# dymensionxyz/cometbft

Measured on AMD Instinct MI355X. Metric: Ed25519 verifs/sec at 1/2/4/8 GPUs + p50 VerifyCommit latency, 150 vals, higher is better.
Workload: dtype u32

## Files before the change

### cometbft_amd/csrc/hs_helper.h

```cpp
#pragma once
#include "devtables.h"
#include "quad.h"

namespace cmtv {

constexpr int kHsCombPre = 6, kHsCombPreFused = 3, kHsCombPreSr = 0;
constexpr uint32_t kHsSlotU2 = 3 * 5 * 64;
constexpr uint32_t kHsTabU2 = 2 * 9 * 5 * 64;

constexpr uint32_t kHsPsWords = 30;
constexpr int kHsFoldCombPre = 15;

__device__ __forceinline__ int hs_comb_pre(uint32_t hs_tune, int dflt) {
  const int c = (hs_tune & 0xFFu) ? (int)(hs_tune & 0xFFu) - 1 : dflt;
  return c > 16 ? 16 : c;
}

__device__ __forceinline__ int hs_workgroup_windows(uint32_t flags, uint32_t t) {
  const bool wide = __ballot(t < 48 && (flags & 2u) != 0) != 0;
  int W = HS_WINDOWS;
#pragma unroll 1
  for (int x = HS_WINDOWS; x < HS_MAX_WINDOWS; x++) W += __ballot(t < 48 && (int)((flags >> 8) & 0xFFu) > x) ? 1 : 0;
  return wide ? HS_WIDE_WINDOWS : W;
}
// ... 3 lines not shown
#pragma unroll
    for (int k = 0; k < 5; k++) dst[(t >> 4) * 320 + k * 64 + 4 * (t & 15) + c] = make_uint2(v.v[2 * k], v.v[2 * k + 1]);
  }
}

__device__ __forceinline__ void hs_slot_store(uint2* dst, uint32_t t, const fe* out) {
#pragma unroll
  for (int c = 0; c < 4; c++) hs_slot_store_coord(dst, t, c, out[c]);
}

struct HsWalk {
  uint32_t tA[8], tR[8];
  const uint2* tw;
  bool r_flip;
  __device__ __forceinline__ HsWalk(const SigPrep& p, int W, const uint2* tabs, uint32_t t) {
    const uint32_t slot = t < 48 ? t : 47;
    r_flip = (p.flags & 1u) != 0;
    hs_digits16(tA, p.k1, W);
    hs_digits16(tR, p.k2, W);
    sc_shift_out(tA, 4);
    sc_shift_out(tR, 4);
    tw = tabs + (slot >> 4) * kHsTabU2 + 4 * (slot & 15);
  }
  __device__ __forceinline__ void next(int& dA, int& dR) {
    dA = (int)sc_shift_out(tA, 4) - 8;
    dR = (int)sc_shift_out(tR, 4) - 8;
  }
  __device__ __forceinline__ void operator()(int P, int e, int c, fe& r) const {
    const uint2* src = tw + (P * 9 + e) * 5 * 64 + c;
#pragma unroll
    for (int k = 0; k < 5; k++) {
      const uint2 x = src[k * 64];
      r.v[2 * k] = x.x;
      r.v[2 * k + 1] = x.y;
    }
  }
};

template <class Clock>
__device__ __forceinline__ void hs_helper_sums(const SigPrep& p, int W, const uint2* tabs, uint2* ring, uint32_t t,
                                               const Clock& clock, uint64_t& hwait) {
  HsWalk rd(p, W, tabs, t);
#pragma unroll 1
  for (int win = W - 2; win >= 0; win--) {
    int dA, dR;
    rd.next(dA, dR);
    fe out[4];
    h_window_addend(out, rd, dA, dR, rd.r_flip);
    hs_slot_store(ring + (win & 1) * kHsSlotU2, t, out);
    const uint64_t c0 = clock();
    __syncthreads();
    hwait += clock() - c0;
  }
}

constexpr uint32_t kHsFgU2 = 2 * 5 * 48;
constexpr uint32_t kHsFgNone = 0xFFFFFFFFu;

__device__ __forceinline__ void hs_helper_sums_fg(const SigPrep& p, int W, const uint2* tabs, uint2* ring, uint2* fg,
                                                  uint32_t* fg_ready, uint32_t t) {
  HsWalk rd(p, W, tabs, t);
#pragma unroll 1
  for (int win = W - 2; win >= 0; win--) {
    int dA, dR;
    rd.next(dA, dR);
    fe z2, f, g;
    h_window_addend_fg(z2, f, g, rd, dA, dR, rd.r_flip);
    if (t < 48) {
#pragma unroll
      for (int k = 0; k < 5; k++) {
        fg[k * 48 + t] = make_uint2(f.v[2 * k], f.v[2 * k + 1]);
        fg[(5 + k) * 48 + t] = make_uint2(g.v[2 * k], g.v[2 * k + 1]);
      }
    }
    hs_slot_store_coord(ring + (win & 1) * kHsSlotU2, t, 2, z2);
    __builtin_amdgcn_fence(__ATOMIC_RELEASE, "workgroup");
    if (t == 0) __hip_atomic_store(fg_ready, (uint32_t)win, __ATOMIC_RELAXED, __HIP_MEMORY_SCOPE_WORKGROUP);
    __syncthreads();
  }
}

template <class Clock>
__device__ __forceinline__ bool hs_helper_sums_eh(const SigPrep& p, int W, const uint2* tabs, uint2* ring,
                                                  const uint2* fg, uint32_t* fg_ready, uint32_t fg_wait, uint32_t t,
                                                  const Clock& clock, uint64_t& hwait, uint64_t& fwait) {
  HsWalk rd(p, W, tabs, t);
  const uint32_t slot = t < 48 ? t : 47;
  bool late = false;
#pragma unroll 1
  for (int win = W - 2; win >= 0; win--) {
    int dA, dR;
    rd.next(dA, dR);
    uint2* dst = ring + (win & 1) * kHsSlotU2;
    fe out[4], e, h;
    h_window_addend_eh(out[3], e, h, rd, dA, dR, rd.r_flip);
    const uint64_t f0 = clock();
    bool ready = false;
    for (uint32_t spins = 0; spins < fg_wait; spins++) {
      ready = __hip_atomic_load(fg_ready, __ATOMIC_RELAXED, __HIP_MEMORY_SCOPE_WORKGROUP) == (uint32_t)win;
      if (ready) break;
      __builtin_amdgcn_s_sleep(1);
    }
    fwait += clock() - f0;
    if (__builtin_expect(__ballot(ready) != __ballot(1), 0)) {
      late = true;
      h_window_addend(out, rd, dA, dR, rd.r_flip);
// ... 48 lines not shown
```

### cometbft_amd/csrc/kernels.h

```cpp
#pragma once
#include <hip/hip_runtime.h>
#include <stdint.h>

namespace cmtv {

constexpr uint32_t kBtabWords = (3 * 128 + 3 * 32768 + 16 * 32768) * 36;
constexpr uint32_t kAtabWordsPerLane = 320;
constexpr uint32_t kCombWords = 32 * 128 * 32;
constexpr uint32_t kCombScratchWordsPerKey = 128 * 320;

constexpr uint32_t kFormLane = 0, kFormQuad = 1, kFormOct2 = 2, kFormRow = 3, kFormRow4 = 4;
constexpr uint32_t kFormMask = 0xFF, kLaunchForceWide = 0x100, kLaunchHsFold = 0x200;
constexpr uint32_t kHsTuneSumSplit = 1u << 11, kHsTuneFgLate = 1u << 12;
constexpr uint32_t kKeyedRow = 0, kKeyedQuad = 1, kKeyedLane = 2;

constexpr uint32_t kRowSlots = 256, kRowSlotWords = 1024, kRowMaxCap = 4 * (kRowSlotWords - 16);
struct RowSlot {
  uint32_t* words = nullptr;
  uint64_t* tagged = nullptr;
  uint32_t seq = 0;
};

struct SbFuse {
  const void* tmpls = nullptr;
  const uint8_t* blob = nullptr;
  const uint32_t* tidx = nullptr;
  const uint8_t* flag = nullptr;
  const int64_t* sec = nullptr;
  const int32_t* nanos = nullptr;
};
constexpr uint32_t kSbFuseMaxMsg = 192;

constexpr uint32_t kDiagLateK = 0, kDiagLatePs = 1, kDiagLateSum = 2, kDiagWords = 4;
constexpr uint32_t kKeyedWaitDefault = 1u << 22, kPsWaitDefault = 1u << 22;

hipError_t launch_btab_init(uint32_t* d_rows, hipStream_t s);
hipError_t launch_verify(uint32_t mode, uint32_t n, const void* pk, const void* sig, const void* msg,
                         const void* off, const uint32_t* btab, uint32_t* atab, void* valid, void* bitmap,
                         uint32_t kflags, hipStream_t s, const SbFuse* sb = nullptr, const RowSlot* row_slot = nullptr,
                         uint32_t ps_wait = kPsWaitDefault, uint32_t* diag = nullptr);
hipError_t launch_comb_build(uint32_t n_keys, const void* keys_pk, uint8_t* keys_ok, uint32_t* tabs,
                             uint32_t* scratch, bool negate, hipStream_t s);
hipError_t launch_verify_keyed(uint32_t mode, uint32_t n, uint32_t n_keys, const void* key_idx, const void* sig,
                               const void* msg, const void* off, const uint32_t* keys_pk, const uint8_t* keys_ok,
                               const uint32_t* ktabs, void* valid, void* bitmap, uint32_t form, uint32_t k_wait,
                               uint32_t* diag, uint32_t batch_kb, uint32_t* scr, const uint32_t* wtabs,
                               const uint32_t* btab, hipStream_t s, const RowSlot* row_slot = nullptr,
                               const SbFuse* sb = nullptr);
hipError_t launch_verify_keyed_lane(uint32_t mode, uint32_t n, uint32_t n_keys, const uint32_t* ki,
                                    const uint32_t* sgp, const uint8_t* mp, const uint32_t* op,
                                    const uint32_t* keys_pk, const uint8_t* keys_ok, const uint32_t* ktabs,
                                    uint8_t* vp, uint64_t* bp, uint32_t batch_kb, uint32_t* scr,
                                    const uint32_t* wtabs, const uint32_t* btab, hipStream_t s);
constexpr size_t kWideTableWords = (size_t)16 * 32768 * 32;
constexpr size_t kWideScratchWordsPerKey = (size_t)16 * (32768 / 64) * 64 * 10;
constexpr size_t kWideBaseWordsPerKey = 16 * 40;
hipError_t launch_wide_build(uint32_t n_keys, const void* keys_pk, uint32_t* tabs, uint32_t* bases,
                             uint32_t* scratch, hipStream_t s);
constexpr uint32_t kKeyedBatchScratchWordsPerSig = 40;
hipError_t launch_verify_sr25519(uint32_t n, const void* pk, const void* sig, const void* msg, const void* off,
                                 const uint32_t* btab, uint32_t* atab, const uint32_t* prog, int nops, void* valid,
                                 void* bitmap, uint32_t kflags, hipStream_t s);
constexpr uint32_t kSecpGtabWords = 33 * 128 * 32;
constexpr uint32_t kSecpQtabWordsPerLane = 240;
hipError_t launch_secp_gtab_build(uint32_t* d_rows, hipStream_t s);
hipError_t launch_verify_secp256k1(uint32_t n, const void* pk, const void* sig, const void* msg, const void* off,
// ... 53 lines not shown
```

### cometbft_amd/csrc/kernels.hip

```cpp
#include <hip/hip_runtime.h>

#include "devtables.h"
#include "hs_helper.h"
#include "kernel_parts.h"
#include "kernels.h"
#include "phase_probe.h"
#include "quad.h"
#include "signbytes.h"
#include "verify_core.h"

CMTV_PHASE_BUFFER()

#ifndef CMTV_QUAD_WAVES_PER_EU
#define CMTV_QUAD_WAVES_PER_EU 1
#endif

#ifndef CMTV_VERIFY_WAVES_PER_EU
#define CMTV_VERIFY_WAVES_PER_EU 2
#endif

namespace cmtv {

template <uint32_t MODE>
__global__ __launch_bounds__(64, CMTV_VERIFY_WAVES_PER_EU) void k_verify(uint32_t n, const uint32_t* __restrict__ pk,
// ... 42 lines not shown
                    [] { CMTV_STAMP(7); });
    const int W = hs_workgroup_windows(p.flags, t);
    p.flags |= (uint32_t)W << 16;
    if (t < 48) sig_prep_store(prep[t], p);
    BComb16 bc;
    bc.init(p.u);
    const DevBTab bt{btab};
#pragma unroll 1
    for (int k = 0; k < comb_pre; k++) bc.step(bt);
    CMTV_STAMP(1);
    __syncthreads();
    CMTV_STAMP(2);
    uint64_t hwait = 0;
    hs_helper_windows(p, W, bc, &tab_lds[0][0], xbuf, t, [] { return (uint64_t)CMTV_CLOCK(); }, hwait);
    CMTV_STAMP_VAL(6, hwait);
    CMTV_STAMP(3);
    __syncthreads();
    return;
  }
  const uint32_t ls = wave * 16 + (t >> 2);
  const uint32_t s = base + ls;
  const bool active = s < n;
  const uint32_t i = active ? s : n - 1;
  DevQuad q;
  DevATabQ ta{tab_lds[wave], t}, tr{tab_lds[wave] + 9 * 5 * 64, t};
  uint64_t qwait = 0;
  (void)qwait;
  DevBTabQ bt{btab};
  bool v = q_verify_hs<MODE>(
      q, pk + 8 * (size_t)i, sig + 16 * (size_t)i, bt, ta, tr, 16 - comb_pre,
      [&](SigPrep& p) {
        CMTV_STAMP(1);
        __syncthreads();
        CMTV_STAMP(2);
        sig_prep_load(p, prep[ls]);
      },
      [&](int win, fe& c) {
        const uint64_t c0 = CMTV_CLOCK();
        __syncthreads();
        qwait += CMTV_CLOCK() - c0;
        hs_slot_load(xbuf + (win & 1) * kHsSlotU2, wave, t, c);
      },
      [&](fe& c) {
        CMTV_STAMP(3);
        __syncthreads();
        CMTV_STAMP(4);
        hs_slot_load(xbuf + kHsSlotU2, wave, t, c);
      });
  CMTV_STAMP(5);
  CMTV_STAMP_VAL(6, qwait);
  quad_verdict_store(v, active, s, n, wave, t, out_valid, out_bitmap, tags);
}

template <uint32_t MODE>
__global__ __launch_bounds__(320, 1) void k_verify_quad_hs_fold(
    uint32_t n, const uint32_t* __restrict__ pk, const uint32_t* __restrict__ sig, const uint8_t* __restrict__ msg,
    const uint32_t* __restrict__ off, const uint32_t* __restrict__ btab, uint8_t* __restrict__ out_valid,
    uint64_t* __restrict__ out_bitmap, uint32_t force_wide, SbFuse sb, uint32_t hs_tune, uint32_t ps_wait,
    uint32_t* __restrict__ diag, RowSlot tags) {
  CMTV_URGENT();
  const uint32_t hw = threadIdx.x >> 6, t = threadIdx.x & 63;
  const uint32_t base = blockIdx.x * 48;
  const uint32_t tune = hs_tune >> 8;
  const int comb_pre = hs_comb_pre(hs_tune, kHsFoldCombPre);
  const uint32_t helper_wave = (tune & 1u) ? 3u : 0u;
  const bool sum_split = (hs_tune & kHsTuneSumSplit) != 0 && helper_wave == 0;
  const bool fg_late = (hs_tune & kHsTuneFgLate) != 0;
  __shared__ uint32_t prep[48][SIG_PREP_WORDS + 1];
  __shared__ uint2 tab_lds[3][kHsTabU2];
  __shared__ uint2 xbuf[2 * kHsSlotU2];
  __shared__ uint32_t ps_ready;
  __shared__ uint2 fgx[kHsFgU2];
  __shared__ uint32_t fg_ready;
  static_assert(sizeof(xbuf) >= 48 * (kSbFuseMaxMsg + 4 * kHsPsWords), "P_s goes behind the sign-bytes buffer");
  static_assert(sizeof(prep) + sizeof(tab_lds) + sizeof(xbuf) + sizeof(fgx) + 2 * sizeof(uint32_t) <= 160 * 1024,
                "a workgroup's LDS");
  uint32_t* pspt = reinterpret_cast<uint32_t*>(xbuf) + 48 * (kSbFuseMaxMsg / 4);
  CMTV_STAMP5(0);
  CMTV_HWID5();
  if (threadIdx.x == 0) {
    ps_ready = 0u;
    fg_ready = kHsFgNone;
  }
  __syncthreads();
  if (hw == 4) {
    if (tune & 2u) __builtin_amdgcn_s_setprio(0);
    if (tune & 4u) __builtin_amdgcn_s_setprio(3);
    if (ps_wait != 0) {
      const uint32_t slot = t < 48 ? t : 47;
      const uint32_t s = base + slot;
      const uint32_t i = s < n ? s : n - 1;
      uint32_t sw[8];
      load_words(sw, sig + 16 * (size_t)i + 8, 2);
      const DevBTab bt{btab};
      BComb16Ahead bc;
      bc.init(sw, bt);
#pragma unroll 1
      for (int k = 0; k < comb_pre; k++) bc.step(bt);
      if (t < 48) {
#pragma unroll
        for (int j = 0; j < 10; j++) {
          pspt[t * kHsPsWords + j] = bc.P.X.v[j];
          pspt[t * kHsPsWords + 10 + j] = bc.P.Y.v[j];
          pspt[t * kHsPsWords + 20 + j] = bc.P.Z.v[j];
        }
      }
      __builtin_amdgcn_fence(__ATOMIC_RELEASE, "workgroup");
      if (t == 0) __hip_atomic_store(&ps_ready, 1u, __ATOMIC_RELAXED, __HIP_MEMORY_SCOPE_WORKGROUP);
    }
    CMTV_STAMP5(3);
    CMTV_STAMP5(1);
    __syncthreads();
    CMTV_STAMP5(2);
    const int W = (int)__builtin_amdgcn_readfirstlane((prep[0][24] >> 16) & 0xFFu);
    if (sum_split && !fg_late) {
      SigPrep p;
      sig_prep_load_pair(p, prep[t < 48 ? t : 47]);
      hs_helper_sums_fg(p, W, &tab_lds[0][0], xbuf, fgx, &fg_ready, t);
      return;
    }
#pragma unroll 1
    for (int win = W - 2; win >= 0; win--) __syncthreads();
    return;
  }
  if (hw == helper_wave) {
    const uint32_t slot = t < 48 ? t : 47;
    const uint32_t s = base + slot;
    const uint32_t i = s < n ? s : n - 1;
    const uint8_t* mp;
    uint32_t ml;
    helper_message(sb, i, msg, off, reinterpret_cast<uint32_t*>(xbuf) + slot * (kSbFuseMaxMsg / 4), mp, ml);
    SigPrep p;
    q_prepare<MODE>(p, pk + 8 * (size_t)i, sig + 16 * (size_t)i, mp, ml, force_wide != 0);
    const int W = hs_workgroup_windows(p.flags, t);
    p.flags |= (uint32_t)W << 16;
    if (t < 48) sig_prep_store_pair(prep[t], p);
    CMTV_STAMP5(1);
    __syncthreads();
    CMTV_STAMP5(2);
    uint64_t hwait = 0, fwait = 0;
    (void)fwait;
    auto clock = [] { return (uint64_t)CMTV_CLOCK(); };
    if (sum_split) {
      const bool late = hs_helper_sums_eh(p, W, &tab_lds[0][0], xbuf, fgx, &fg_ready, fg_late ? 0u : kPsWaitDefault, t,
                                          clock, hwait, fwait);
      if (late && t == 0 && diag) atomicAdd(diag + kDiagLateSum, 1u);
    } else {
      hs_helper_sums(p, W, &tab_lds[0][0], xbuf, t, clock, hwait);
    }
    CMTV_STAMP5_VAL(4, fwait);
    CMTV_STAMP5_VAL(7, hwait);
    CMTV_STAMP5(3);
    return;
  }
  const uint32_t wave = hw - (hw > helper_wave ? 1u : 0u);
  const uint32_t ls = wave * 16 + (t >> 2);
  const uint32_t s = base + ls;
  const bool active = s < n;
  const uint32_t i = active ? s : n - 1;
  DevQuad q;
  DevATabQ ta{tab_lds[wave], t}, tr{tab_lds[wave] + 9 * 5 * 64, t};
  uint64_t qwait = 0;
  (void)qwait;
  bool v = q_verify_hs_fold<MODE>(
      q, pk + 8 * (size_t)i, sig + 16 * (size_t)i, DevBTabQ{btab}, 16 - comb_pre, ta, tr,
      [&](fe& ps) {
        const uint64_t c0 = CMTV_CLOCK();
        (void)c0;
        bool ready = false;
        for (uint32_t spins = 0; spins < ps_wait; spins++) {
          ready = __hip_atomic_load(&ps_ready, __ATOMIC_RELAXED, __HIP_MEMORY_SCOPE_WORKGROUP) != 0u;
          if (ready) break;
          __builtin_amdgcn_s_sleep(2);
        }
        CMTV_STAMP5_VAL(3, CMTV_CLOCK() - c0);
        if (__builtin_expect(__ballot(ready) != __ballot(1), 0)) {
          if (t == 0 && diag) atomicAdd(diag + kDiagLatePs, 1u);
          return false;
        }
        __builtin_amdgcn_fence(__ATOMIC_ACQUIRE, "workgroup");
        const int lane = (int)(t & 3);
        const uint32_t* pp = pspt + ls * kHsPsWords;
        fe a, b;
#pragma unroll
        for (int j = 0; j < 10; j++) {
          a.v[j] = pp[10 * q_p2_factor_a(lane) + j];
          b.v[j] = pp[10 * q_p2_factor_b(lane) + j];
        }
        fe_mul(ps, a, b);
        CMTV_STAMP5(4);
        return true;
      },
      [&](SigPrep& p) {
        CMTV_STAMP5(1);
        __syncthreads();
        CMTV_STAMP5(2);
        sig_prep_load_pair(p, prep[ls]);
      },
      [&](int win, fe& c) {
        const uint64_t c0 = CMTV_CLOCK();
        __syncthreads();
        qwait += CMTV_CLOCK() - c0;
        hs_slot_load(xbuf + (win & 1) * kHsSlotU2, wave, t, c);
      });
  CMTV_STAMP5(5);
  CMTV_STAMP5_VAL(7, qwait);
  quad_verdict_store(v, active, s, n, wave, t, out_valid, out_bitmap, tags);
}

template <uint32_t MODE>
__global__ __launch_bounds__(128, CMTV_QUAD_WAVES_PER_EU) void k_verify_oct_split(
    uint32_t n, const uint32_t* __restrict__ pk, const uint32_t* __restrict__ sig, const uint8_t* __restrict__ msg,
    const uint32_t* __restrict__ off, const uint32_t* __restrict__ btab, uint8_t* __restrict__ out_valid,
    uint64_t* __restrict__ out_bitmap, uint32_t force_wide, SbFuse sb) {
  CMTV_URGENT();
  const uint32_t t = threadIdx.x & 63;
  const uint32_t gid = blockIdx.x * 64 + t;
  const uint32_t s = gid >> 3;
  const bool active = s < n;
  const uint32_t i = active ? s : n - 1;
  __shared__ uint32_t prep[8][SIG_PREP_WORDS + 1];
  __shared__ uint32_t bpt[8][40];
  __shared__ uint2 tab_lds[9 * 5 * 64];
  __shared__ uint32_t sbm[8][kSbFuseMaxMsg / 4];
  if (threadIdx.x >= 64) {
    const uint8_t* mp;
    uint32_t ml;
    helper_message(sb, i, msg, off, sbm[t >> 3], mp, ml);
    SigPrep p;
    q_prepare<MODE>(p, pk + 8 * (size_t)i, sig + 16 * (size_t)i, mp, ml, force_wide != 0);
    if ((t & 7) == 0) sig_prep_store(prep[t >> 3], p);
    __syncthreads();
    ge_p3 B;
    q_bcomb16(B, p.u, DevBTab{btab});
    if ((t & 7) == 0) bpoint_store(bpt[t >> 3], B);
    __syncthreads();
    return;
  }
  DevOct q;
  DevBTabQ bt{btab};
  DevATabQ ta{tab_lds, t};
  const uint32_t* bq = &bpt[t >> 3][10 * (t & 3)];
  bool v = o_verify_split<MODE, true>(
      q, pk + 8 * (size_t)i, sig + 16 * (size_t)i, bt, ta,
      [&](SigPrep& p) {
        __syncthreads();
        sig_prep_load(p, prep[t >> 3]);
      },
      [&](fe& c) {
        __syncthreads();
#pragma unroll
        for (int j = 0; j < 10; j++) c.v[j] = bq[j];
      });
  v = v && active;
  if (active && (t & 7) == 0 && out_valid) out_valid[s] = v ? 1 : 0;
  uint64_t x = __ballot(v && (t & 7) == 0) & 0x0101010101010101ull;
  x = (x | (x >> 7)) & 0x0003000300030003ull;
  x = (x | (x >> 14)) & 0x0000000F0000000Full;
  x = (x | (x >> 28)) & 0xFFull;
  if (t == 0 && out_bitmap) reinterpret_cast<uint8_t*>(out_bitmap)[gid >> 6] = (uint8_t)x;
}

// ... 180 lines not shown
  const uint32_t limb = reinterpret_cast<const uint16_t*>(((t >> 4) & 1) ? sgp : pkp)[t & 15];
  DevRowTab tab{tab_lo, t};
  bool a_ok, r_ok, r_canon;
  const uint32_t v = r_sum_ar(x, limb, pkw, sigw, tab, get_prep, kRowLoWindows, p, a_ok, r_ok, r_canon);
  CMTV_STAMP(3);
  __syncthreads();
  CMTV_STAMP(4);
  const uint32_t cb = bpt_limb(bpt, t);
  bool v_ok = r_join4<MODE>(x, v, xh[0][t], xh[1][t], cb, (p.flags & 4u) != 0 && a_ok && r_ok, r_canon);
  CMTV_STAMP(5);
  CMTV_STAMP_RT(6);
  const bool active = s < n;
  v_ok = v_ok && active;
  if (t == 0 && active && out_valid) out_valid[s] = v_ok ? 1 : 0;
  if (out_bitmap && active) row_bitmap_add(slot, s, n, v_ok, out_bitmap, t);
}

hipError_t launch_verify(uint32_t mode, uint32_t n, const void* pk, const void* sig, const void* msg,
                         const void* off, const uint32_t* btab, uint32_t* atab, void* valid, void* bitmap,
                         uint32_t kflags, hipStream_t s, const SbFuse* sb, const RowSlot* row_slot, uint32_t ps_wait,
                         uint32_t* diag) {
  const SbFuse fz = sb ? *sb : SbFuse{};
  const uint32_t form = kflags & kFormMask;
  const uint32_t fw = (kflags & kLaunchForceWide) ? 1u : 0u;
  if (n == 0) return hipSuccess;
  auto pkp = static_cast<const uint32_t*>(pk);
  auto sgp = static_cast<const uint32_t*>(sig);
  auto mp = static_cast<const uint8_t*>(msg);
  auto op = static_cast<const uint32_t*>(off);
  auto vp = static_cast<uint8_t*>(valid);
  auto bp = static_cast<uint64_t*>(bitmap);
  const RowSlot rs = row_slot ? *row_slot : RowSlot{};
  if ((form == kFormRow4 || form == kFormRow) && (n > kRowMaxCap || (bp && !rs.words))) return hipErrorInvalidValue;
  if (form != kFormLane && form != kFormQuad && form != kFormOct2 && form != kFormRow && form != kFormRow4)
    return hipErrorInvalidValue;
  if (fz.tmpls && form == kFormLane) return hipErrorInvalidValue;
  with_mode(mode, [&](auto m) {
    constexpr uint32_t M = decltype(m)::value;
    switch (form) {
      case kFormRow4:
        hipLaunchKernelGGL(k_verify_row4_split<M>, dim3(n), dim3(256), 0, s, n, pkp, sgp, mp, op, btab, vp, bp, fw, fz,
                           rs);
        break;
      case kFormRow:
        hipLaunchKernelGGL(k_verify_row_split<M>, dim3((n + 2) / 3), dim3(256), 0, s, n, pkp, sgp, mp, op, btab, vp, bp,
                           fw, fz, rs);
        break;
      case kFormOct2:
        hipLaunchKernelGGL(k_verify_oct_split<M>, dim3(((n + 63) / 64) * 8), dim3(128), 0, s, n, pkp, sgp, mp, op, btab,
                           vp, bp, fw, fz);
        break;
      case kFormQuad: {
        const uint32_t slices = 4 * ((n + 63) / 64);
        if (kflags & kLaunchHsFold)
          hipLaunchKernelGGL(k_verify_quad_hs_fold<M>, dim3((slices + 2) / 3), dim3(320), 0, s, n, pkp, sgp, mp, op,
                             btab, vp, bp, fw, fz, kflags >> 16, ps_wait, diag, rs);
        else
          hipLaunchKernelGGL(k_verify_quad_hs<M>, dim3((slices + 2) / 3), dim3(256), 0, s, n, pkp, sgp, mp, op, btab,
                             vp, bp, fw, fz, kflags >> 16, rs);
        break;
      }
      default:
        hipLaunchKernelGGL(k_verify<M>, dim3((n + 63) / 64), dim3(64), 0, s, n, pkp, sgp, mp, op, btab, atab, vp, bp);
    }
  });
  return hipGetLastError();
}

}
```

### cometbft_amd/csrc/launch.cpp

```cpp
#include "runtime_state.h"

namespace cmtv {

struct LaunchScope {
  cmtv_ctx* ctx;
  CmtvDev& D;
  hipStream_t s;
  Timing::Pair tp{};
  bool timed = false;
  hipError_t begin() {
    D.timing.harvest(ctx->stats, D.device_ms, D.timed_calls, false);
    timed = ctx->timing_every && D.timing_seq++ % ctx->timing_every == 0;
    return timed ? D.timing.begin(tp, s) : hipSuccess;
  }
  hipError_t launched(hipError_t e) {
    if (e != hipSuccess) {
      D.timing.abandon(tp);
      return e;
    }
    ctx->stats.kernel_launches++;
    D.launches++;
    return hipSuccess;
  }
  int finish(size_t n, Scratch* lane_scratch) {
// ... 11 lines not shown
static void take_tags(CmtvDev& D, RowSlot& slot, uint32_t width) {
  slot.tagged = D.tag_arm;
  slot.seq = D.tag_seq;
  D.tag_used = true;
  D.tag_width = width;
}

bool fault_hit(cmtv_ctx* ctx) {
  ctx->launch_seq++;
  if (ctx->fault_at && ctx->launch_seq == ctx->fault_at) {
    ctx->stats.faults_injected++;
    ctx->fault_pending = true;
    return true;
  }
  return false;
}

static hipError_t row_slot_acquire(cmtv_ctx* ctx, CmtvDev& D, hipStream_t s, bool bitmap, RowSlot& slot,
                                   uint32_t& k) {
  hipError_t e0 = settle_polled(D);
  if (e0 != hipSuccess) return e0;
  k = D.row_seq++ % kRowSlots;
  slot = RowSlot{};
  slot.words = D.d_rowslots + (size_t)k * kRowSlotWords;
  if (bitmap && D.tag_arm) take_tags(D, slot, 32);
  if (!D.row_pending[k] || !ctx->row_fence) return hipSuccess;
  hipError_t e = hipEventQuery(D.row_ev[k]);
  if (e == hipErrorNotReady) e = hipStreamWaitEvent(s, D.row_ev[k], 0);
  if (e != hipSuccess) return e;
  D.row_pending[k] = false;
  return hipSuccess;
}

static hipError_t row_slot_release(cmtv_ctx* ctx, CmtvDev& D, hipStream_t s, uint32_t k) {
  if (ctx->host_sync || !ctx->row_fence) return hipSuccess;
  hipError_t e = hipSuccess;
  if (!D.row_ev[k]) e = hipEventCreateWithFlags(&D.row_ev[k], hipEventDisableTiming);
  if (e == hipSuccess) e = hipEventRecord(D.row_ev[k], s);
  if (e == hipSuccess) D.row_pending[k] = true;
  return e;
}

int enqueue_verify(cmtv_ctx* ctx, CmtvDev& D, size_t n, const uint8_t* d_pk, const uint8_t* d_sig,
                   const uint8_t* d_msg, const uint32_t* d_off, uint32_t mode, uint8_t* d_valid, uint64_t* d_bitmap,
                   hipStream_t s, const SbFuse* sb, Scratch* scr) {
  Scratch& S = scr ? *scr : D.scratch;
  if (n == 0) return CMTV_OK;
  if (fault_hit(ctx) || D.inject_fault) return CMTV_EHIP;
  if (sb && (mode == kModeSr25519 || !fuse_ok(ctx, n))) return CMTV_EINVAL;
  const bool sr = mode == kModeSr25519;
  const uint32_t form = sr ? sr_form(ctx, n) : ed_form(ctx, n);
  const bool lane = form == kFormLane;
  const bool row = form == kFormRow || form == kFormRow4;
  const uint32_t hs_tune = ctx->hs_tune | (ctx->hs_sum_split ? kHsTuneSumSplit : 0u) | (ctx->fg_late ? kHsTuneFgLate : 0u);
  const uint32_t kflags = form | (form == kFormQuad ? hs_tune << 16 : 0u) |
                          (ctx->force_wide ? kLaunchForceWide : 0u) | (ctx->hs_fold ? kLaunchHsFold : 0u);
  hipError_t e = hipSuccess;
  if (lane) {
    const size_t lanes = std::min<size_t>(n, ctx->lane_chunk);
    const size_t lanes_padded = (lanes + 63) / 64 * 64;
    if ((e = acquire_scratch(S, lanes_padded * kAtabWordsPerLane * sizeof(uint32_t), s)) != hipSuccess)
      return hip_fail(e);
  }
  RowSlot slot;
  uint32_t slot_k = 0;
  if (row && (e = row_slot_acquire(ctx, D, s, d_bitmap != nullptr, slot, slot_k)) != hipSuccess) return hip_fail(e);
  const bool qtag = ctx->quad_poll && !sr && form == kFormQuad && d_bitmap && D.tag_arm && n <= kChunk;
  if (qtag) {
    slot = RowSlot{};
    take_tags(D, slot, 16);
  }
  LaunchScope L{ctx, D, s};
  if ((e = L.begin()) != hipSuccess) return hip_fail(e);
  const size_t chunk = lane ? ctx->lane_chunk : kChunk;
  for (size_t c = 0; c < n; c += chunk) {
    const uint32_t cn = (uint32_t)std::min<size_t>(chunk, n - c);
    if (sr)
      e = launch_verify_sr25519(cn, d_pk + 32 * c, d_sig + 64 * c, d_msg, d_off + c, D.d_btab,
                                static_cast<uint32_t*>(S.buf.p), D.d_srprog, ctx->sr_nops,
                                d_valid ? d_valid + c : nullptr, d_bitmap ? d_bitmap + c / 64 : nullptr, kflags, s);
    else
      e = launch_verify(mode, cn, d_pk + 32 * c, d_sig + 64 * c, d_msg, d_off + c, D.d_btab,
                        static_cast<uint32_t*>(S.buf.p), d_valid ? d_valid + c : nullptr,
                        d_bitmap ? d_bitmap + c / 64 : nullptr, kflags, s, sb, row || qtag ? &slot : nullptr,
                        ctx->ps_wait, D.d_diag);
    if (e == hipSuccess && row) e = row_slot_release(ctx, D, s, slot_k);
    if ((e = L.launched(e)) != hipSuccess) return hip_fail(e);
  }
  return L.finish(n, lane ? &S : nullptr);
}

int enqueue_verify_keyed(cmtv_ctx* ctx, CmtvDev& D, const cmtv_keyset::PerDev& K, size_t n_keys, size_t n,
                         const uint32_t* d_idx, const uint8_t* d_sig, const uint8_t* d_msg, const uint32_t* d_off,
                         uint32_t mode, uint8_t* d_valid, uint64_t* d_bitmap, hipStream_t s, Scratch* scr,
                         const SbFuse* sb, uint32_t min_waves) {
  if (n == 0) return CMTV_OK;
  if (!min_waves) min_waves = ctx->keyed_batch_min_waves;
  Scratch& S = scr ? *scr : D.scratch;
  if (sb && !keyed_fuse_ok(ctx, n)) return CMTV_EINVAL;
  if (!d_idx && !sb) return CMTV_EINVAL;
  if (fault_hit(ctx) || D.inject_fault) return CMTV_EHIP;
  const uint32_t form = keyed_form(ctx, n);
  const bool batch = form == kKeyedLane;
  const size_t chunk = batch ? kKeyedBatchChunk : kChunk;
  auto kb_for = [&](size_t cn) -> uint32_t { return batch ? keyed_batch_kb(cn, min_waves) : 1; };
  hipError_t e;
  const uint32_t kb0 = kb_for(std::min(chunk, n));
// ... 151 lines not shown
```

### cometbft_amd/csrc/quad.h

```cpp
#pragma once
#include "halfscalar.h"
#include "verify_core.h"

namespace cmtv {

constexpr int QP_B0 = 0x00, QP_B1 = 0x55, QP_B2 = 0xAA, QP_B3 = 0xFF;
constexpr int QP_SWAP01 = (1 << 0) | (0 << 2) | (2 << 4) | (3 << 6);

constexpr int qp(int s0, int s1, int s2, int s3) { return s0 | (s1 << 2) | (s2 << 4) | (s3 << 6); }

CMTV_HD uint32_t fe_p2(int i) { return i == 0 ? P2_0 : ((i & 1) ? P2_O : P2_E); }

CMTV_HD void fe_pick(fe& h, int lane, const fe& a, const fe& b, const fe& c, const fe& d) {
  const bool l1 = lane & 1, l2 = lane & 2;
#pragma unroll
  for (int i = 0; i < 10; i++) {
    const uint32_t lo = l1 ? b.v[i] : a.v[i];
    const uint32_t hi = l1 ? d.v[i] : c.v[i];
    h.v[i] = l2 ? hi : lo;
  }
}

CMTV_HD void q_identity(fe& v, int lane) {
  fe_0(v);
// ... 644 lines not shown
  rd(0, eA, 1, y);
  fe_sub(d, y, x);
  fe_add(s, y, x);
  rd(1, eR, 0, x);
  rd(1, eR, 1, y);
  fe_sub(d2, y, x);
  fe_add(s2, y, x);
  fe_select(x, d, s, nA);
  fe_select(m, d2, s2, nR);
  fe_mul(x, x, m);
  fe_select(y, s, d, nA);
  fe_select(m, s2, d2, nR);
  fe_mul(y, y, m);
  fe_sub(e, y, x);
  fe_add(h, y, x);
  fe T3;
  fe_mul(T3, e, h);
  fe_const_d2(m);
  fe_mul(out3, T3, m);
}

template <class Rd>
CMTV_HD void h_window_addend_fg(fe& out2, fe& f, fe& g, const Rd& rd, int dA, int dR, bool r_flip) {
  const int eA = dA < 0 ? -dA : dA, eR = dR < 0 ? -dR : dR;
  const bool nA = dA < 0, nR = (dR < 0) != r_flip;
  fe x, y, s, d, m, d2;
  rd(1, eR, 3, m);
  fe_const_d2(d2);
  fe_mul(m, m, d2);
  rd(0, eA, 3, x);
  fe_mul(x, x, m);
  rd(0, eA, 2, y);
  rd(1, eR, 2, m);
  fe_add(m, m, m);
  fe_mul(y, y, m);
  fe_add(s, y, x);
  fe_sub(d, y, x);
  const bool cneg = nA != nR;
  fe_select(f, d, s, cneg);
  fe_select(g, s, d, cneg);
  fe Z3;
  fe_mul(Z3, f, g);
  fe_add(out2, Z3, Z3);
}

CMTV_HD void h_window_addend_xy(fe& out0, fe& out1, const fe& e, const fe& f, const fe& g, const fe& h) {
  fe X3, Y3;
  fe_mul(X3, e, f);
  fe_mul(Y3, g, h);
  fe_sub(out0, Y3, X3);
  fe_add(out1, Y3, X3);
}

template <class Q, class BTab, class ATab, class GetPrep, class GetS, class GetB>
CMTV_HD void q_hs_straus(const Q& q, fe& v, fe& rc, const BTab& btab, ATab& tabA, ATab& tabR, int j0, SigPrep& p,
                         const GetPrep& get_prep, const GetS& get_s, const GetB& get_b) {
  const int lane = q.lane();
  q_build_table_p3(q, tabA, v);
  q_build_table_p3(q, tabR, rc);
  get_prep(p);
  const bool r_flip = (p.flags & 1u) != 0;
  const int W = (p.flags >> 16) & 0xFFu ? (int)((p.flags >> 16) & 0xFFu) : q_wave_windows(q, p.flags);
  uint32_t tA[8], tR[8];
  hs_digits16(tA, p.k1, W);
  hs_digits16(tR, p.k2, W);
  uint32_t tLo[8], tHi[8];
  hs_digits65536(tLo, tHi, p.u);
#pragma unroll 1
  for (int j = 15; j >= j0; j--) sc_shift_out(j >= 8 ? tHi : tLo, 16);
  fe c;
  {
    const int dA = (int)sc_shift_out(tA, 4) - 8;
    const int dR = (int)sc_shift_out(tR, 4) - 8;
    tabA.load(dA < 0 ? -dA : dA, v);
    fe t, r;
    fe_neg(t, v);
    fe_carry(t);
    fe_select(v, v, t, dA < 0 && (lane == 0 || lane == 3));
    tabR.load(dR < 0 ? -dR : dR, r);
    fe_neg(t, r);
    fe_carry(t);
    fe_select(r, r, t, ((dR < 0) != r_flip) && (lane == 0 || lane == 3));
    q_to_cached(q, c, r);
    q_add(q, v, c);
  }
#pragma unroll 1
  for (int win = W - 2; win >= 0; win--) {
    const bool hi = (win & 2) != 0;
    const bool has_b = (win & 1) == 0 && win <= 30 && (hi ? 8 : 0) + (win >> 2) < j0;
    bool b_neg = false, b_ident = false;
    fe cB;
    if (has_b) {
      const int dB = (int)sc_shift_out(hi ? tHi : tLo, 16) - 0x8000;
      const int ib = dB < 0 ? -dB : dB;
      const int row = BT16_BASE + (ib > 0 ? ib - 1 : 0) + (hi ? BT16_ENTRIES : 0);
      q_niels_load(
          q, cB, [&](int off, fe& r) { btab.load_coord(row, off, r); }, BTAB_COORD_WORDS, 2 * BTAB_COORD_WORDS,
          dB < 0);
      b_neg = dB < 0;
      b_ident = ib == 0;
    }
#pragma unroll 1
    for (int d = 0; d < 4; d++) q_dbl(q, v);
    get_s(win, c);
    q_add(q, v, c);
    if (has_b) {
// ... 174 lines not shown
```

### cometbft_amd/csrc/runtime.cpp

```cpp
#include <climits>
#include <cstdio>
#include <cstdlib>
#include <new>
#include <thread>

#include "runtime_state.h"
#include "merlin.h"

namespace cmtv {

uint64_t phase_now(const cmtv_ctx* ctx) { return phase_clock(ctx); }

void phase_add(cmtv_ctx* ctx, int phase, uint64_t t0) {
  if (!ctx->phases_on || !t0) return;
  ctx->phase_ns[phase] += phase_clock(ctx) - t0;
  if (phase == kPhPrepare) ctx->phase_calls++;
}

void phase_add_ns(cmtv_ctx* ctx, int phase, uint64_t ns) {
  if (!ctx->phases_on) return;
  ctx->phase_ns[phase] += ns;
  if (phase == kPhPipePlan) ctx->phase_calls++;
}

// ... 145 lines not shown
    if (q == std::string::npos) q = list.size();
    const std::string tok = list.substr(p, q - p);
    p = q + 1;
    if (tok.empty()) continue;
    bool known = false;
    for (const auto& k : kNames)
      if (tok == k.name) {
        (k.keyed ? ctx->force_keyed : ctx->force_form) = k.form;
        known = true;
      }
    if (!known) std::fprintf(stderr, "cmtverify: CMTV_FORM: unknown form '%s' ignored\n", tok.c_str());
  }
}

static void env_is(const char* name, char c, bool& flag) {
  if (const char* v = std::getenv(name)) flag = v[0] == c;
}
static void env_not(const char* name, char c, bool& flag) {
  if (const char* v = std::getenv(name)) flag = v[0] != c;
}
template <class T>
static void env_int(const char* name, long lo, long hi, T& field) {
  const char* v = std::getenv(name);
  if (!v) return;
  const long x = std::strtol(v, nullptr, 10);
  if (x >= lo && x <= hi) field = (T)x;
}

static void read_env(cmtv_ctx* ctx) {
  if (const char* f = std::getenv("CMTV_FORM")) parse_forms(ctx, f);
  if (const char* hp = std::getenv("CMTV_HS_PRE")) {
    char* end = nullptr;
    const long v = std::strtol(hp, &end, 10);
    if (end != hp && *end == 0 && v >= 0 && v <= 16) ctx->hs_tune = (uint32_t)(v + 1);
  }
  if (const char* lc = std::getenv("CMTV_LANE_CHUNK")) {
    const size_t v = (size_t)std::strtoull(lc, nullptr, 10) / 64 * 64;
    if (v >= 64 && v <= kChunk) ctx->lane_chunk = v;
  }
  if (const char* sm = std::getenv("CMTV_SHARD_MIN")) ctx->shard_min = (size_t)std::strtoull(sm, nullptr, 10);
  if (const char* fa = std::getenv("CMTV_FAULT_AT")) ctx->fault_at = (uint64_t)std::strtoull(fa, nullptr, 10);
  env_is("CMTV_FORCE_WIDE", '1', ctx->force_wide);
  env_not("CMTV_NO_SB_FUSE", '1', ctx->sb_fuse);
  env_not("CMTV_NO_ZC_IN", '1', ctx->zc_in);
  env_not("CMTV_ZC_HOST_IN", '0', ctx->zc_host_in);
  env_not("CMTV_EARLY_SIGS", '0', ctx->early_sigs);
  if (const char* hp = std::getenv("CMTV_HOST_POLL")) ctx->host_poll = std::atoi(hp) != 0;
  if (const char* kl = std::getenv("CMTV_FORCE_K_LATE")) ctx->keyed_wait = kl[0] == '1' ? 0u : kKeyedWaitDefault;
  env_not("CMTV_HS_FOLD", '0', ctx->hs_fold);
  if (const char* pl = std::getenv("CMTV_FORCE_PS_LATE")) ctx->ps_wait = pl[0] == '1' ? 0u : kPsWaitDefault;
  env_not("CMTV_HS_SUM_SPLIT", '0', ctx->hs_sum_split);
  env_is("CMTV_FORCE_FG_LATE", '1', ctx->fg_late);
  if (ctx->fg_late && !std::getenv("CMTV_HS_SUM_SPLIT")) ctx->hs_sum_split = true;
  {
    uint32_t ft = 0;
    env_int("CMTV_HS_FOLD_TUNE", 0, 7, ft);
    ctx->hs_tune |= ft << 8;
  }
  env_int("CMTV_KEYED_BATCH_MIN_WAVES", 1, 1l << 20, ctx->keyed_batch_min_waves);
  env_int("CMTV_KEYED_BATCH_MIN_WAVES", 1, 1l << 20, ctx->secp_batch_min_waves);
  if (std::getenv("CMTV_KEYED_BATCH_MIN_WAVES")) ctx->secp_batch_max_kb = 8;
  env_not("CMTV_ROW_FENCE", '0', ctx->row_fence);
  env_is("CMTV_HOST_PHASES", '1', ctx->phases_on);
  if (const char* tm = std::getenv("CMTV_TIMING")) {
    const long v = std::strtol(tm, nullptr, 10);
    ctx->timing_every = v < 0 ? 0u : (uint32_t)std::min<long>(v, 1l << 20);
  }
  if (const char* fs = std::getenv("CMTV_FAULT_SYNC_DEV")) {
    char* end = nullptr;
    const long g = std::strtol(fs, &end, 10);
    if (end != fs && g >= 0) ctx->fault_sync_dev = g;
  }
  ctx->force_rccl = std::getenv("CMTV_FORCE_RCCL") != nullptr;
  if (const char* rl = std::getenv("CMTV_RCCL_LIB")) ctx->rccl_lib = rl;
  ctx->no_rccl = std::getenv("CMTV_NO_RCCL") != nullptr;
  ctx->no_rccl_fallback = std::getenv("CMTV_NO_RCCL_FALLBACK") != nullptr;
  env_int("CMTV_HOST_THREADS", 1, 256, ctx->host_threads);
  if (const char* v = std::getenv("CMTV_PIPE_MIN")) ctx->pipe_min = (size_t)std::strtoull(v, nullptr, 10);
  if (const char* v = std::getenv("CMTV_PIPE_CHUNK")) {
    const size_t c = (size_t)std::strtoull(v, nullptr, 10);
    if (c >= 64 && c <= (1u << 24)) ctx->pipe_chunk = c;
  }
  env_int("CMTV_PIPE_SLOTS", 2, kBulkSlotsMax, ctx->pipe_slots);
  env_not("CMTV_PIPELINE", '0', ctx->pipe_on);
  env_not("CMTV_PIPE_DIRECT", '0', ctx->pipe_direct);
  env_int("CMTV_SPEC_MIN", 1, LONG_MAX, ctx->spec_min);
  if (const char* v = std::getenv("CMTV_SPEC")) {
    if (v[0] == '0') ctx->spec_min = 0;
  }
  if (const char* v = std::getenv("CMTV_LAT_WINDOW_MS")) ctx->lat_window_ns = 1'000'000ull * std::strtoull(v, nullptr, 10);
  env_not("CMTV_LOAD_FORM", '0', ctx->load_form);
  env_not("CMTV_LOAD_ZC", '0', ctx->load_zc);
  env_is("CMTV_LOAD_POLL", '0', ctx->load_nopoll);
  env_is("CMTV_QUAD_POLL", '1', ctx->quad_poll);
  env_not("CMTV_KEYED_ZC", '0', ctx->keyed_zc);
  env_is("CMTV_SPIN_WAIT", '1', ctx->spin_wait);
  env_not("CMTV_PREP_STREAM", '0', ctx->prep_stream);
  env_is("CMTV_ONE_EXEC", '1', ctx->one_exec);
  env_is("CMTV_BULK_BM_DIRECT", '1', ctx->bulk_bm_direct);
  env_not("CMTV_SPLIT_SUBMIT", '0', ctx->split_submit);
  if (const char* v = std::getenv("CMTV_CALL_TRACE")) {
    ctx->call_trace = v[0] == '1' || v[0] == '2';
    ctx->call_trace_loaded_only = v[0] == '2';
  }
  env_not("CMTV_LAT_ISOLATE", '0', ctx->lat_isolate);
  env_int("CMTV_LAT_RESERVE_CUS", 1, 64, ctx->lat_reserve_cus);
// ... 491 lines not shown
```

### cometbft_amd/csrc/runtime_state.h

```cpp
#pragma once
#include <hip/hip_runtime.h>

#include <algorithm>
#include <array>
#include <atomic>
#include <chrono>
#include <cstring>
#include <deque>
#include <map>
#include <memory>
#include <mutex>
#include <random>
#include <string>
#include <unordered_map>
#include <vector>

#include "../../include/cmtverify.h"
#include "host_pool.h"
#include "kernels.h"
#include "runtime_internal.h"

namespace cmtv {

constexpr uint32_t kChunk = 1u << 18;
// ... 220 lines not shown
  int ordinal = 0;
  hipStream_t stream = nullptr;
  uint32_t* d_btab = nullptr;
  uint32_t* d_srprog = nullptr;
  uint32_t* d_secp_gtab = nullptr;
  DevBuf secp_in, secp_out;
  std::vector<uint8_t> secp_stage;
  MerkleSlot merkle[2];
  DevBuf d_in, d_out, d_all;
  HostBuf h_in, h_out;
  HostBuf h_zc{nullptr, 0, hipHostMallocCoherent | hipHostMallocMapped};
  HostBuf h_zin{nullptr, 0, hipHostMallocCoherent | hipHostMallocMapped};
  Scratch scratch;
  hipEvent_t done = nullptr;
  Timing timing;
  ncclComm_t comm = nullptr;
  uint32_t* d_diag = nullptr;
  uint32_t* d_rowslots = nullptr;
  uint32_t row_seq = 0;
  hipEvent_t row_ev[cmtv::kRowSlots] = {};
  bool row_pending[cmtv::kRowSlots] = {};
  HostBuf h_tags{nullptr, 0, hipHostMallocCoherent | hipHostMallocMapped};
  uint64_t* d_tags = nullptr;
  uint64_t* tag_arm = nullptr;
  uint32_t tag_seq = 0;
  bool tag_used = false;
  uint32_t tag_width = 32;
  hipEvent_t poll_ev = nullptr;
  bool poll_pending = false;
  const uint8_t* early_src = nullptr;
  const uint8_t* early_pk = nullptr;
  size_t early_n = 0;
  bool failed = false;
  bool inject_fault = false;
  uint64_t calls = 0, signatures = 0, launches = 0, timed_calls = 0;
  double device_ms = 0;
  uint64_t timing_seq = 0;
  BulkLane bulk;
};

}

struct cmtv_ctx {
  std::vector<cmtv::CmtvDev> devs;
  bool rccl = false;
  uint32_t default_mode = CMTV_MODE_GO_STDLIB;
  std::mutex mu;
  cmtv_stats stats{};
  uint32_t force_form = cmtv::kNoForm, force_keyed = cmtv::kNoForm;
  uint32_t hs_tune = 0;
  bool hs_fold = true;
  uint32_t ps_wait = cmtv::kPsWaitDefault;
  bool hs_sum_split = false, fg_late = false;
  uint64_t late_sum_waves = 0;
  size_t lane_chunk = cmtv::kChunk;
  size_t shard_min = cmtv::kShardMinDefault;
  int sr_nops = 0;
  cmtv::VerdictCache cache;
  size_t keyset_cap = 0;
  std::vector<std::pair<std::string, cmtv_keyset*>> keysets;
  std::vector<cmtv_secp_keyset*> secp_keysets;
  uint64_t fault_at = 0, launch_seq = 0;
  bool fault_pending = false;
  bool force_rccl = false, no_rccl = false, no_rccl_fallback = false;
  std::string rccl_lib;
  bool rccl_broken = false;
  uint32_t rccl_drain_ms = 2000;
  bool force_wide = false;
  bool sb_fuse = true;
  uint32_t keyed_wait = cmtv::kKeyedWaitDefault;
  uint32_t keyed_batch_min_waves = cmtv::kKeyedBatchMinWaves;
  uint32_t secp_batch_min_waves = cmtv::kSecpBatchMinWaves;
  uint32_t secp_batch_max_kb = cmtv::kSecpBatchMaxKb;
  std::vector<size_t> live;
  bool zc_in = true;
  bool zc_host_in = true;
  bool early_sigs = true;
  size_t zc_max = cmtv::kZeroCopyMax;
  bool host_poll = true;
  bool host_sync = false;
  bool row_fence = true;
  uint32_t timing_every = 16;
  bool phases_on = false;
  uint64_t phase_ns[cmtv::kPhCount] = {};
  uint64_t phase_calls = 0;
  long fault_sync_dev = -1;
  std::mutex bulk_mu;
  std::unique_ptr<cmtv::HostPool> pool;
  unsigned host_threads = 0;
  size_t pipe_min = 32768, pipe_chunk = 1u << 20;
  int pipe_slots = 3;
  bool pipe_on = true;
  bool pipe_direct = true;
  std::atomic<uint64_t> last_latency_ns{0};
  bool load_form = true;
  bool bulk_now = false, load_zc = true;
  bool load_nopoll = true;
  bool quad_poll = false;
  bool keyed_zc = true;
  bool spin_wait = false;
  bool prep_stream = true;
  bool one_exec = false;
  bool bulk_bm_direct = false;
  bool split_submit = true;
  bool call_trace = false, call_trace_loaded_only = false;
  uint64_t trace_launch = 0, trace_wait = 0;
// ... 146 lines not shown
```

Measured before the change: 51.27 million.

## Pipeline helper window sums across lead and helper waves in hs_fold kernel

Adds a pipelined window-addend path for the quad hs_fold kernel. Each window's addend computation is split into a front half (table reads plus the first multiplies) and a back half (the final products), and the two halves are spread across the lead wave and the helper waves on alternating windows. The lead wave raises its scheduling priority and signals urgency after the first window. The intent is to shorten the per-window critical path between barriers. It is enabled by default through a new env flag and template parameter, and it adds more register state and a dependence on the barrier cadence.

```diff
diff --git a/cometbft_amd/csrc/hs_helper.h b/cometbft_amd/csrc/hs_helper.h
--- a/cometbft_amd/csrc/hs_helper.h
+++ b/cometbft_amd/csrc/hs_helper.h
@@ -79,6 +79,21 @@
     __syncthreads();
     hwait += clock() - c0;
   }
+}
+
+template <class Clock, class FirstDone>
+__device__ __forceinline__ void hs_helper_sums_pipe(const SigPrep& p, int W, const uint2* tabs, uint2* ring,
+                                                    uint32_t t, bool lead, const Clock& clock, uint64_t& hwait,
+                                                    const FirstDone& first_done) {
+  HsWalk rd(p, W, tabs, t);
+  h_sums_pipe(
+      rd, W, lead, [&](int win, const fe* out) { hs_slot_store(ring + (win & 1) * kHsSlotU2, t, out); },
+      [&](int win) {
+        const uint64_t c0 = clock();
+        __syncthreads();
+        hwait += clock() - c0;
+        if (win == W - 2) first_done();
+      });
 }
 
 constexpr uint32_t kHsFgU2 = 2 * 5 * 48;
diff --git a/cometbft_amd/csrc/kernels.h b/cometbft_amd/csrc/kernels.h
--- a/cometbft_amd/csrc/kernels.h
+++ b/cometbft_amd/csrc/kernels.h
@@ -12,6 +12,7 @@
 constexpr uint32_t kFormLane = 0, kFormQuad = 1, kFormOct2 = 2, kFormRow = 3, kFormRow4 = 4;
 constexpr uint32_t kFormMask = 0xFF, kLaunchForceWide = 0x100, kLaunchHsFold = 0x200;
 constexpr uint32_t kHsTuneSumSplit = 1u << 11, kHsTuneFgLate = 1u << 12;
+constexpr uint32_t kHsTunePipe = 1u << 13;
 constexpr uint32_t kKeyedRow = 0, kKeyedQuad = 1, kKeyedLane = 2;
 
 constexpr uint32_t kRowSlots = 256, kRowSlotWords = 1024, kRowMaxCap = 4 * (kRowSlotWords - 16);
diff --git a/cometbft_amd/csrc/kernels.hip b/cometbft_amd/csrc/kernels.hip
--- a/cometbft_amd/csrc/kernels.hip
+++ b/cometbft_amd/csrc/kernels.hip
@@ -118,7 +118,7 @@
   quad_verdict_store(v, active, s, n, wave, t, out_valid, out_bitmap, tags);
 }
 
-template <uint32_t MODE>
+template <uint32_t MODE, bool PIPE>
 __global__ __launch_bounds__(320, 1) void k_verify_quad_hs_fold(
     uint32_t n, const uint32_t* __restrict__ pk, const uint32_t* __restrict__ sig, const uint8_t* __restrict__ msg,
     const uint32_t* __restrict__ off, const uint32_t* __restrict__ btab, uint8_t* __restrict__ out_valid,
@@ -179,6 +179,15 @@
     __syncthreads();
     CMTV_STAMP5(2);
     const int W = (int)__builtin_amdgcn_readfirstlane((prep[0][24] >> 16) & 0xFFu);
+    if constexpr (PIPE) {
+      SigPrep p;
+      sig_prep_load_pair(p, prep[t < 48 ? t : 47]);
+      uint64_t hwait = 0;
+      hs_helper_sums_pipe(
+          p, W, &tab_lds[0][0], xbuf, t, false, [] { return (uint64_t)CMTV_CLOCK(); }, hwait, [] {});
+      CMTV_STAMP5_VAL(7, hwait);
+      return;
+    }
     if (sum_split && !fg_late) {
       SigPrep p;
       sig_prep_load_pair(p, prep[t < 48 ? t : 47]);
@@ -207,7 +216,10 @@
     uint64_t hwait = 0, fwait = 0;
     (void)fwait;
     auto clock = [] { return (uint64_t)CMTV_CLOCK(); };
-    if (sum_split) {
+    if constexpr (PIPE) {
+      __builtin_amdgcn_s_setprio(3);
+      hs_helper_sums_pipe(p, W, &tab_lds[0][0], xbuf, t, true, clock, hwait, [] { CMTV_URGENT(); });
+    } else if (sum_split) {
       const bool late = hs_helper_sums_eh(p, W, &tab_lds[0][0], xbuf, fgx, &fg_ready, fg_late ? 0u : kPsWaitDefault, t,
                                           clock, hwait, fwait);
       if (late && t == 0 && diag) atomicAdd(diag + kDiagLateSum, 1u);
@@ -274,6 +286,10 @@
   quad_verdict_store(v, active, s, n, wave, t, out_valid, out_bitmap, tags);
 }
 
+static bool hs_fold_pipe(uint32_t hs_tune) {
+  return (hs_tune & kHsTunePipe) != 0 && (hs_tune & kHsTuneSumSplit) == 0 && ((hs_tune >> 8) & 1u) == 0;
+}
+
 template <uint32_t MODE>
 __global__ __launch_bounds__(128, CMTV_QUAD_WAVES_PER_EU) void k_verify_oct_split(
     uint32_t n, const uint32_t* __restrict__ pk, const uint32_t* __restrict__ sig, const uint8_t* __restrict__ msg,
@@ -560,9 +576,12 @@
         break;
       case kFormQuad: {
         const uint32_t slices = 4 * ((n + 63) / 64);
-        if (kflags & kLaunchHsFold)
-          hipLaunchKernelGGL(k_verify_quad_hs_fold<M>, dim3((slices + 2) / 3), dim3(320), 0, s, n, pkp, sgp, mp, op,
-                             btab, vp, bp, fw, fz, kflags >> 16, ps_wait, diag, rs);
+        if ((kflags & kLaunchHsFold) && hs_fold_pipe(kflags >> 16))
+          hipLaunchKernelGGL((k_verify_quad_hs_fold<M, true>), dim3((slices + 2) / 3), dim3(320), 0, s, n, pkp, sgp, mp,
+                             op, btab, vp, bp, fw, fz, kflags >> 16, ps_wait, diag, rs);
+        else if (kflags & kLaunchHsFold)
+          hipLaunchKernelGGL((k_verify_quad_hs_fold<M, false>), dim3((slices + 2) / 3), dim3(320), 0, s, n, pkp, sgp, mp,
+                             op, btab, vp, bp, fw, fz, kflags >> 16, ps_wait, diag, rs);
         else
           hipLaunchKernelGGL(k_verify_quad_hs<M>, dim3((slices + 2) / 3), dim3(256), 0, s, n, pkp, sgp, mp, op, btab,
                              vp, bp, fw, fz, kflags >> 16, rs);
diff --git a/cometbft_amd/csrc/launch.cpp b/cometbft_amd/csrc/launch.cpp
--- a/cometbft_amd/csrc/launch.cpp
+++ b/cometbft_amd/csrc/launch.cpp
@@ -87,7 +87,8 @@
   const uint32_t form = sr ? sr_form(ctx, n) : ed_form(ctx, n);
   const bool lane = form == kFormLane;
   const bool row = form == kFormRow || form == kFormRow4;
-  const uint32_t hs_tune = ctx->hs_tune | (ctx->hs_sum_split ? kHsTuneSumSplit : 0u) | (ctx->fg_late ? kHsTuneFgLate : 0u);
+  const uint32_t hs_tune = ctx->hs_tune | (ctx->hs_sum_split ? kHsTuneSumSplit : 0u) |
+                           (ctx->fg_late ? kHsTuneFgLate : 0u) | (ctx->hs_sum_pipe ? kHsTunePipe : 0u);
   const uint32_t kflags = form | (form == kFormQuad ? hs_tune << 16 : 0u) |
                           (ctx->force_wide ? kLaunchForceWide : 0u) | (ctx->hs_fold ? kLaunchHsFold : 0u);
   hipError_t e = hipSuccess;
diff --git a/cometbft_amd/csrc/quad.h b/cometbft_amd/csrc/quad.h
--- a/cometbft_amd/csrc/quad.h
+++ b/cometbft_amd/csrc/quad.h
@@ -720,6 +720,84 @@
   fe_add(out1, Y3, X3);
 }
 
+template <class Rd>
+CMTV_HD void h_window_addend_front(fe& e, fe& f, fe& g, fe& h, const Rd& rd, int dA, int dR, bool r_flip) {
+  const int eA = dA < 0 ? -dA : dA, eR = dR < 0 ? -dR : dR;
+  const bool nA = dA < 0, nR = (dR < 0) != r_flip;
+  fe x, y, s, d, m, s2, d2;
+  rd(0, eA, 0, x);
+  rd(0, eA, 1, y);
+  fe_sub(d, y, x);
+  fe_add(s, y, x);
+  rd(1, eR, 0, x);
+  rd(1, eR, 1, y);
+  fe_sub(d2, y, x);
+  fe_add(s2, y, x);
+  fe_select(x, d, s, nA);
+  fe_select(m, d2, s2, nR);
+  fe_mul(x, x, m);
+  fe_select(y, s, d, nA);
+  fe_select(m, s2, d2, nR);
+  fe_mul(y, y, m);
+  fe_sub(e, y, x);
+  fe_add(h, y, x);
+  rd(1, eR, 3, m);
+  fe_const_d2(d2);
+  fe_mul(m, m, d2);
+  rd(0, eA, 3, x);
+  fe_mul(x, x, m);
+  rd(0, eA, 2, y);
+  rd(1, eR, 2, m);
+  fe_add(m, m, m);
+  fe_mul(y, y, m);
+  fe_add(s, y, x);
+  fe_sub(d, y, x);
+  const bool cneg = nA != nR;
+  fe_select(f, d, s, cneg);
+  fe_select(g, s, d, cneg);
+}
+
+CMTV_HD void h_window_addend_back(fe out[4], const fe& e, const fe& f, const fe& g, const fe& h) {
+  fe X3, Y3, Z3, T3, m;
+  fe_mul(X3, e, f);
+  fe_mul(Y3, g, h);
+  fe_mul(Z3, f, g);
+  fe_mul(T3, e, h);
+  fe_sub(out[0], Y3, X3);
+  fe_add(out[1], Y3, X3);
+  fe_add(out[2], Z3, Z3);
+  fe_const_d2(m);
+  fe_mul(out[3], T3, m);
+}
+
+CMTV_HD bool h_sums_pipe_owns(int W, int win, bool lead) { return (((W - 2 - win) & 1) == 0) == lead; }
+
+template <class Walk, class Store, class Barrier>
+CMTV_HD void h_sums_pipe(Walk& rd, int W, bool lead, const Store& store, const Barrier& barrier) {
+  fe e, f, g, h;
+  int dA, dR;
+  auto front = [&] {
+    rd.next(dA, dR);
+    h_window_addend_front(e, f, g, h, rd, dA, dR, rd.r_flip);
+    rd.next(dA, dR);
+  };
+  if (lead)
+    front();
+  else
+    rd.next(dA, dR);
+#pragma unroll 1
+  for (int win = W - 2; win >= 0; win--) {
+    if (h_sums_pipe_owns(W, win, lead)) {
+      fe out[4];
+      h_window_addend_back(out, e, f, g, h);
+      store(win, out);
+    } else if (win > 0) {
+      front();
+    }
+    barrier(win);
+  }
+}
+
 template <class Q, class BTab, class ATab, class GetPrep, class GetS, class GetB>
 CMTV_HD void q_hs_straus(const Q& q, fe& v, fe& rc, const BTab& btab, ATab& tabA, ATab& tabR, int j0, SigPrep& p,
                          const GetPrep& get_prep, const GetS& get_s, const GetB& get_b) {
diff --git a/cometbft_amd/csrc/runtime.cpp b/cometbft_amd/csrc/runtime.cpp
--- a/cometbft_amd/csrc/runtime.cpp
+++ b/cometbft_amd/csrc/runtime.cpp
@@ -221,6 +221,7 @@
   env_not("CMTV_HS_SUM_SPLIT", '0', ctx->hs_sum_split);
   env_is("CMTV_FORCE_FG_LATE", '1', ctx->fg_late);
   if (ctx->fg_late && !std::getenv("CMTV_HS_SUM_SPLIT")) ctx->hs_sum_split = true;
+  env_not("CMTV_HS_SUM_PIPE", '0', ctx->hs_sum_pipe);
   {
     uint32_t ft = 0;
     env_int("CMTV_HS_FOLD_TUNE", 0, 7, ft);
diff --git a/cometbft_amd/csrc/runtime_state.h b/cometbft_amd/csrc/runtime_state.h
--- a/cometbft_amd/csrc/runtime_state.h
+++ b/cometbft_amd/csrc/runtime_state.h
@@ -296,6 +296,7 @@
   bool hs_fold = true;
   uint32_t ps_wait = cmtv::kPsWaitDefault;
   bool hs_sum_split = false, fg_late = false;
+  bool hs_sum_pipe = true;
   uint64_t late_sum_waves = 0;
   size_t lane_chunk = cmtv::kChunk;
   size_t shard_min = cmtv::kShardMinDefault;
```

Result: faster. 52.39 million (median of 6 runs) (+2.2%).
